# daooshee/ReReVST-Code

Measured on AMD Instinct MI355X. Metric: stylized frames/sec at 512x512, 1 style, higher is better.
Workload: dtype f32

## Files before the change

rerevst-code_amd/build.py:

```python
import os
import subprocess
import sys

HERE = os.path.dirname(os.path.abspath(__file__))
CSRC = os.path.join(HERE, "csrc")
LIB = os.path.join(HERE, "librerevst_hip.so")
SOURCES = ["rerevst_hip.hip"]
HEADERS = ["conv_mfma.h", "conv_wino.h", "conv_wino_split.h", "conv_f43.h", "conv_thin.h", "prep_kernels.h", "../../include/rerevst_hip.h"]


def _stale():
    if not os.path.exists(LIB):
        return True
    t = os.path.getmtime(LIB)
    return any(os.path.getmtime(os.path.join(CSRC, f)) > t for f in SOURCES + HEADERS)


def build_lib(force=False, verbose=True, extra=()):
    if not force and not _stale():
        return LIB
    hipcc = os.environ.get("HIPCC", "/opt/rocm/bin/hipcc")
    cmd = [hipcc, "--offload-arch=gfx950", "-O3", "-std=c++17", "-shared", "-fPIC",
           "-Wno-unused-result", *extra,
           *[os.path.join(CSRC, s) for s in SOURCES], "-o", LIB]
# ... 9 lines not shown
```

rerevst-code_amd/csrc/conv_wino.h:

```cpp
#pragma once
#include <hip/hip_runtime.h>
#include <stdint.h>
#include <utility>
#include <type_traits>
#include "conv_mfma.h"

#define WINO_PAR_BYTES 2048

template <int NW, int UPS, int SC = 0>
struct WinoGeo {
    static constexpr int NT = NW * 64;
    static constexpr int NB = NW == 8 ? 1 : 2;
    static constexpr int NP = UPS ? 9 : 16;
    static constexpr int NPU = NP + SC;
    static constexpr int PW = UPS ? 3 : 4;
    static constexpr int NPIECE = PW * PW;
    static constexpr int PPI = UPS ? 3 : 2;
    static constexpr int TIN = UPS ? 8 : 16;
    static constexpr int HALO = UPS ? 10 : 18;
    static constexpr int HALF = 18 * 9;
    static constexpr int PIECES = HALO * HALO * 4;
    static constexpr int RAW_IT = (PIECES + NT - 1) / NT;
    static constexpr int RAW_BYTES = RAW_IT * NT * 16;
    static constexpr int U_BYTES = NPU * 32 * 16 * 4;
    static constexpr int U_PIECES = U_BYTES / 16;
    static constexpr int U_IT = (U_PIECES + NT - 1) / NT;
    static constexpr int U_LDS = U_IT * NT * 16;
    static constexpr int SMEM = 2 * RAW_BYTES + 2 * U_LDS + WINO_PAR_BYTES;
    static constexpr int OCC = (UPS && NW == 4) ? 2 : 1;
// ... 83 lines not shown
    return r;
}
__device__ __forceinline__ f32x4 f4norm_clamp(const f32x4 v, const f32x4 m, const f32x4 r, const f32x4 lo, const f32x4 hi) {
    const f32x4 n = e4mul(f4sub(v, m), r);
    f32x4 o;
#pragma unroll
    for (int e = 0; e < 4; ++e) o[e] = med3(n[e], lo[e], hi[e]);
    return o;
}

template <class F, int... I>
__device__ __forceinline__ void static_for(F&& f, std::integer_sequence<int, I...>) {
    (f(std::integral_constant<int, I>{}), ...);
}

template <int EPI, int ABL = 0, int NW = 4, int UPS = 1, int SC = 0, int PERIMG = 0>
__global__ __launch_bounds__(NW * 64, (WinoGeo<NW, UPS, SC>::OCC)) void conv_wino_k(const ConvP p) {
    static_assert(UPS == 1 && NW == 4, "library kernel: upsample-fused form, 4 waves");
    static_assert(!(EPI & E_POOL), "no pooling behind an upsample");
    using G = WinoGeo<NW, UPS, SC>;
    constexpr int NPU = G::NPU;
    constexpr int RAW_BYTES = G::RAW_BYTES, U_BYTES = G::U_BYTES, U_LDS = G::U_LDS, NT = G::NT, NB = G::NB, NP = G::NP, PW = G::PW, NPIECE = G::NPIECE;
    extern __shared__ __attribute__((aligned(16))) char smem[];
    const int tid = threadIdx.x;
    const int wave = __builtin_amdgcn_readfirstlane(tid >> 6);
    const int lane = tid & 63, t = lane & 15, q = lane >> 4;
    const int tr = t >> 3, tc = t & 7;
    const int tg = wave;
    const int nchunks = p.Cin >> 4;
    const int n_ntiles = p.Cout >> 5;

    struct Item { int tx, ty, b, nt; };
    Item cur, nxt, dlt;
    {
        const int GD = gridDim.x, w = blockIdx.x;
// ... 100 lines not shown
        constexpr int PAR = decltype(par_c)::value;
        constexpr bool FIRST = decltype(first_c)::value;
        const bool own_u = c + 1 < nchunks, own_r = c + 2 < nchunks;
        const rsrc_t rs_u = make_rsrc(own_u ? w_t : w_n);
        const rsrc_t rs_ul = make_rsrc(own_u ? w_t : w_n, u_last_num);
        const rsrc_t rs_r = make_rsrc(own_r ? in_t : in_n);
        const rsrc_t rs_rl = make_rsrc(own_r ? in_t : in_n, raw_last_num);
        const int usoff = own_u ? (c + 1) * U_BYTES : 0;
        const int rsoff = (own_r ? c + 2 : c + 2 - nchunks) * 64;
        char* const udst = smem + 2 * RAW_BYTES + (1 - PAR) * U_LDS;
        char* const rdst = smem + PAR * RAW_BYTES;
        if (ABL & 128) {
            f32x4 u01[2] = {vcur[0], vcur[1]};
#pragma unroll
            for (int i = 0; i < NPU; ++i) {
                const f32x4 vv = vcur[i < NP ? i : 0];
#pragma unroll
                for (int s = 0; s < 4; ++s)
#pragma unroll
                    for (int nb = 0; nb < NB; ++nb)
                        acc[i][nb] = __builtin_amdgcn_mfma_f32_16x16x4f32(u01[nb][s], vv[s], (FIRST && s == 0) ? f32x4{0.f, 0.f, 0.f, 0.f} : acc[i][nb], 0, 0, 0);
            }
#pragma unroll
            for (int i = 0; i < NPIECE; ++i) vnext[i] = vcur[i];
            return;
        }
        const unsigned ub = PAR ? offU1 : offU;
        constexpr int RB = (1 - PAR) * RAW_BYTES;
        f32x4 u[4][NB];
        f32x4 (&d)[NPIECE] = vnext;
        u[0][0] = lds_rd128<0>(ub);
// ... 12 lines not shown
            }, std::make_integer_sequence<int, G::PPI>{});
            constexpr int cdx = i - 3;
            static_assert(G::col_iter(0) == 3 && G::col_iter(PW - 1) == PW + 2, "column release schedule");
            if constexpr (cdx >= 0 && cdx < PW) {
                asm volatile("s_waitcnt lgkmcnt(%5)" : "+v"(d[cdx * 3 + 0]), "+v"(d[cdx * 3 + 1]), "+v"(d[cdx * 3 + 2]), "+v"(u[i & 3][0]), "+v"(u[i & 3][1]) : "i"(G::younger(i)));
            } else {
                lds_release2<G::younger(i)>(u[i & 3][0], u[i & 3][1]);
            }
            __builtin_amdgcn_sched_barrier(0);
            if (!(ABL & 1)) {
                {
                    if constexpr (i < G::U_IT) bufld16_rs(i == G::U_IT - 1 ? rs_ul : rs_u, udst + (i * NT + wave * 64) * 16, tid * 16, usoff + i * NT * 16);
                    if constexpr (i < G::RAW_IT) bufld16_rs(i == G::RAW_IT - 1 ? rs_rl : rs_r, rdst + (i * NT + wave * 64) * 16, asrc[i], rsoff);
                }
            }
            const f32x4 vv = vcur[i < NP ? (i % PW) * PW + i / PW : 0];
#pragma unroll
            for (int s = 0; s < 4; ++s)
#pragma unroll
                for (int nb = 0; nb < NB; ++nb)
                    acc[i][nb] = __builtin_amdgcn_mfma_f32_16x16x4f32(u[i & 3][nb][s], vv[s], (FIRST && s == 0) ? f32x4{0.f, 0.f, 0.f, 0.f} : acc[i][nb], 0, 0, 0);
            static_for([&](auto xc) {
                constexpr int k = decltype(xc)::value;
                if constexpr (G::col_iter(k) == i) col_pass(d, k);
                if constexpr (G::row_iter(k) == i) row_pass(d, k);
            }, std::make_integer_sequence<int, PW>{});
        }, std::make_integer_sequence<int, NPU>{});
    };

    int par_ntile = -1, par_img = -1;
    long long tl[6] = {0, 0, 0, 0, 0, 0}, tl_t = 0;
// ... 53 lines not shown
        const int yb = e_y0 + 4 * tg + 2 * tr, xb = e_x0 + 2 * tc;
        f32x4 resv[NB][2][2];
        if (EPI & (E_RES | E_RES_UPS)) {
#pragma unroll
            for (int nb = 0; nb < NB; ++nb)
#pragma unroll
                for (int i = 0; i < 2; ++i)
#pragma unroll
                    for (int j = 0; j < 2; ++j) {
                        const int y = yb + i, x = xb + j;
                        const int ry = (EPI & E_RES_UPS) ? (y >> 1) : y, rx = (EPI & E_RES_UPS) ? (x >> 1) : x;
                        resv[nb][i][j] = f32x4{0.f, 0.f, 0.f, 0.f};
                        if (y < p.H && x < p.W)
                            resv[nb][i][j] = *(const f32x4*)(res_b + ((ry + 1) * (p.Wr + 2) + rx + 1) * p.Cout + e_ntile * 32 + nb * 16 + 4 * q);
                    }
        }
        if constexpr (SC) {
            const int ly = yb >> 1, lx = xb >> 1;
            if (ly < p.Hi && lx < p.Wi) {
                float* sc_b = p.sc_out + (size_t)e_b * (size_t)(p.Hi + 2) * (p.Wi + 2) * p.Cout + ((size_t)(ly + 1) * (p.Wi + 2) + lx + 1) * p.Cout;
#pragma unroll
                for (int nb = 0; nb < NB; ++nb) *(f32x4*)(sc_b + e_ntile * 32 + nb * 16 + 4 * q) = acc[NP][nb];
            }
        }
#pragma unroll
        for (int nb = 0; nb < NB; ++nb) {
            const int co = e_ntile * 32 + nb * 16 + 4 * q;
            f32x4 Y[2][2];
            f32x4 T[2][3];
#pragma unroll
            for (int c = 0; c < 3; ++c) {
                T[0][c] = acc[0 + c][nb] + acc[3 + c][nb];
                T[1][c] = acc[0 + c][nb] + acc[6 + c][nb];
            }
#pragma unroll
            for (int i = 0; i < 2; ++i) {
                Y[i][0] = T[i][0] + T[i][1];
                Y[i][1] = T[i][0] + T[i][2];
// ... 26 lines not shown
                        else if (p.out_p8) *(f32x4*)(out_b + (size_t)(co >> 3) * ((size_t)(p.H + 2) * (p.W + 8) * 8) + ((size_t)(y + 1) * (p.W + 8) + x + 4) * 8 + (co & 7)) = o;
                        else *(f32x4*)(out_b + ((y + 1) * (p.W + 2) + x + 1) * p.Cout + co) = o;
                    }
                }
        }
        tick(5);
    }
    asm volatile("s_waitcnt vmcnt(0)" ::: "memory");
    if ((ABL & 16) && lane == 0) {
        long long* dbg = p.dbg;
#pragma unroll
        for (int k = 0; k < 6; ++k) dbg[(blockIdx.x * NW + wave) * 6 + k] = tl[k];
    }
}

__global__ void pack_wino_k(const float* __restrict__ w, float* __restrict__ dst, int Cout, int Cin, int ups,
                            const float* __restrict__ wsc = nullptr) {
    constexpr int CH = 16;
    const int npt = ups ? 9 : 16, pw = ups ? 3 : 4;
    const int np = npt + (wsc ? 1 : 0);
    const size_t total = (size_t)Cout * Cin * np;
    for (size_t i = blockIdx.x * (size_t)blockDim.x + threadIdx.x; i < total; i += (size_t)gridDim.x * blockDim.x) {
        size_t r = i;
        const int cl = (int)(r % CH); r /= CH;
        const int j = r & 31; r >>= 5;
        const int pos = (int)(r % np); r /= np;
        const int nchunks = Cin / CH;
        const int chunk = r % nchunks; r /= nchunks;
        const int n_tile = (int)r;
        const int e = cl & 3, qs = cl >> 2;
        const int qq = qs ^ ((0 - (j >> 2)) & 3);
        const int co = n_tile * 32 + j, ci = chunk * CH + qq * 4 + e;
        if (pos >= npt) { dst[i] = wsc[(size_t)co * Cin + ci]; continue; }
        const float* g = w + ((size_t)co * Cin + ci) * 9;
        const int pr = pos / pw, pc = pos % pw;
        auto G3 = [&](int row, float g0, float g1, float g2) {
            if (ups) return row == 0 ? g0 + g1 + g2 : (row == 1 ? g0 : g2);
            return row == 0 ? g0 : (row == 1 ? 0.5f * (g0 + g1 + g2) : (row == 2 ? 0.5f * (g0 - g1 + g2) : g2));
        };
        float rowv[3];
#pragma unroll
        for (int kx = 0; kx < 3; ++kx) rowv[kx] = G3(pr, g[0 * 3 + kx], g[1 * 3 + kx], g[2 * 3 + kx]);
        dst[i] = G3(pc, rowv[0], rowv[1], rowv[2]);
    }
}
```

rerevst-code_amd/csrc/rerevst_hip.hip:

```cpp
#include <hip/hip_runtime.h>
#include <dlfcn.h>
#include <stddef.h>
#include <stdint.h>
#include <string.h>
#include <algorithm>
#include <cmath>
#include <thread>
#include <stdio.h>
#include <map>
#include <condition_variable>
#include <mutex>
#include <string>
#include <vector>

#include "../../include/rerevst_hip.h"
#include "conv_mfma.h"
#include "conv_wino.h"
#include "conv_wino_split.h"
#include "conv_f43.h"
#include "conv_thin.h"
#include "prep_kernels.h"

namespace {

// ... 380 lines not shown
    hipLaunchKernelGGL((conv_mfma_k<BN, TAPS, EPI>), grid, dim3(256), 0, s, p);
}

typedef void (*ConvFn)(const ConvP&, dim3, hipStream_t);
typedef hipError_t (*AttrFn)();
struct ConvKey { int BN, TAPS, UPS, EPI; ConvFn fn; const char* name; AttrFn attr; ConvFn fn_img = nullptr; };
#define CK(BN, TAPS, UPS, EPI) {BN, TAPS, UPS, EPI, &conv_launch<BN, TAPS, EPI>, "conv_mfma<" #BN "," #TAPS "," #EPI ">", nullptr}
const ConvKey CONV_TABLE[] = {
    CK(128, 1, 0, 0), CK(64, 1, 0, 0),
    CK(32, 9, 0, 0),
    CK(64, 9, 0, E_RELU | E_POOL), CK(128, 9, 0, E_RELU), CK(128, 9, 0, E_RELU | E_POOL), CK(128, 9, 0, E_RELU | E_NORM1),
};

constexpr int WINO_NW = 8;
constexpr int UPW_NW = 4;
template <int EPI, int NW, int UPS, int SC, int PERIMG = 0>
void wino_launch(const ConvP& p, dim3 grid, hipStream_t s) {
    using Geo = WinoGeo<NW, UPS, SC>;
    hipLaunchKernelGGL((conv_wino_k<EPI, 0, NW, UPS, SC, PERIMG>), grid, dim3(NW * 64), Geo::SMEM, s, p);
}
template <int EPI, int NW, int UPS, int SC, int PERIMG = 0>
hipError_t wino_attr() {
    hipError_t e = hipFuncSetAttribute((const void*)conv_wino_k<EPI, 0, NW, UPS, SC, 0>, hipFuncAttributeMaxDynamicSharedMemorySize, WinoGeo<NW, UPS, SC>::SMEM);
    if (e == hipSuccess && PERIMG) e = hipFuncSetAttribute((const void*)conv_wino_k<EPI, 0, NW, UPS, SC, 1>, hipFuncAttributeMaxDynamicSharedMemorySize, WinoGeo<NW, UPS, SC>::SMEM);
    return e;
}
template <int EPI, int PERIMG>
void wsplit_launch(const ConvP& p, dim3 grid, hipStream_t s) {
    hipLaunchKernelGGL((conv_wino_split_k<EPI, PERIMG>), grid, dim3(512), WSPLIT_SMEM_BYTES, s, p);
}
template <int EPI, int PERIMG>
hipError_t wsplit_attr() {
    hipError_t e = hipFuncSetAttribute((const void*)conv_wino_split_k<EPI, 0>, hipFuncAttributeMaxDynamicSharedMemorySize, WSPLIT_SMEM_BYTES);
    if (e == hipSuccess && PERIMG) e = hipFuncSetAttribute((const void*)conv_wino_split_k<EPI, 1>, hipFuncAttributeMaxDynamicSharedMemorySize, WSPLIT_SMEM_BYTES);
    return e;
}
template <int EPI, int LAY = 0>
void f43_launch(const ConvP& p, dim3 grid, hipStream_t s) {
    hipLaunchKernelGGL((conv_f43_k<EPI, LAY>), grid, dim3(F43Geo::NT), F43Geo::SMEM, s, p);
}
template <int EPI, int LAY = 0>
hipError_t f43_attr() { return hipFuncSetAttribute((const void*)conv_f43_k<EPI, LAY>, hipFuncAttributeMaxDynamicSharedMemorySize, F43Geo::SMEM); }
#define FK(EPI) {32, 9, 0, EPI, &f43_launch<EPI>, "conv_f43<" #EPI ">", &f43_attr<EPI>, nullptr}
struct F43LayKey { int EPI, LAY; ConvFn fn; const char* name; AttrFn attr; };
#define FKL(EPI, LAY) {EPI, LAY, &f43_launch<EPI, LAY>, "conv_f43<" #EPI ", " #LAY ">", &f43_attr<EPI, LAY>}
#define WK(EPI) {32, 9, 0, EPI, &wsplit_launch<EPI, 0>, "conv_wino<" #EPI ">", &wsplit_attr<EPI, 0>, nullptr}
#define WKI(EPI) {32, 9, 0, EPI, &wsplit_launch<EPI, 0>, "conv_wino<" #EPI ">", &wsplit_attr<EPI, 1>, &wsplit_launch<EPI, 1>}
#define UW(EPI) {32, 9, 1, EPI, &wino_launch<EPI, UPW_NW, 1, 0>, "conv_upw<" #EPI ">", &wino_attr<EPI, UPW_NW, 1, 0>}
#define UWS(EPI) {32, 10, 1, EPI, &wino_launch<EPI, UPW_NW, 1, 1>, "conv_upw_sc<" #EPI ">", &wino_attr<EPI, UPW_NW, 1, 1>}
#define UWSI(EPI) {32, 10, 1, EPI, &wino_launch<EPI, UPW_NW, 1, 1>, "conv_upw_sc<" #EPI ">", &wino_attr<EPI, UPW_NW, 1, 1, 1>, &wino_launch<EPI, UPW_NW, 1, 1, 1>}
const ConvKey WINO_TABLE[] = {
    WK(E_RELU), WK(E_RELU | E_POOL), WK(E_RELU | E_NORM1), WKI(E_LRELU | E_NORM1 | E_RES_UPS | E_NORM2), WKI(E_LRELU),
    WKI(0),
    WKI(E_RES), WKI(E_RES | E_NORM2),
    UW(E_LRELU | E_NORM1), UW(E_LRELU),
    UWSI(E_LRELU | E_NORM1),
    UWS(E_LRELU),
};

const ConvKey F43_TABLE[] = { FK(E_RELU), FK(E_RELU | E_POOL), FK(E_RELU | E_NORM1), FK(E_LRELU | E_NORM1 | E_RES_UPS | E_NORM2) };
const F43LayKey F43_LAY_TABLE[] = {
    FKL(E_RELU | E_POOL, 3), FKL(E_RELU, 3),
    FKL(E_RELU | E_POOL, 1),
    FKL(E_LRELU | E_NORM1 | E_RES_UPS | E_NORM2, 1),
};
// ... 26 lines not shown
int conv(rrv_handle h, const ConvCall& c) {
    const ConvW& w = *c.w;
    const ConvKey* k = nullptr;
    bool wino = false;
    bool f43 = !c.direct && use_f43(h, w, c.B, c.H, c.W, c.epi, c.ups, c.ksplit, c.bias_bstride != 0 || c.w_bstride != 0) &&
               !((c.wy0 | c.wx0 | c.wy1 | c.wx1) & 31);
    if (f43) {
        f43 = false;
        for (const ConvKey& e : F43_TABLE)
            if (e.EPI == c.epi) { k = &e; f43 = true; wino = true; break; }
    }
    const bool fuse_sc = c.ups && c.sc_out != nullptr;
    if (fuse_sc && !w.pk_ups_sc) return fail(h, RRV_E_ARG, "conv: no shortcut-fused pack for this layer");
    if (!f43 && !c.direct && (c.ups ? w.pk_ups != nullptr : w.pk_wino != nullptr)) {
        for (const ConvKey& e : WINO_TABLE)
            if (e.EPI == c.epi && e.UPS == (int)c.ups && (e.TAPS == 10) == fuse_sc) { k = &e; wino = true; break; }
    }
    const int ks = c.ksplit > 1 ? c.ksplit : 1;
    if (ks > 1 && !(wino && !c.ups && w.Cout == 32 && (w.Cin % (32 * ks)) == 0 && c.bias))
        return fail(h, RRV_E_ARG, "conv: split K needs the row-split kernel, a 32-cout layer, an even number of 16-channel chunks per slice and a split bias");
    if (!k && !c.ups) {
        for (const ConvKey& e : CONV_TABLE)
            if (e.BN == w.BN && e.TAPS == w.taps && e.EPI == c.epi) { k = &e; break; }
    }
    if (!k) {
        char b[128];
        snprintf(b, sizeof b, "no conv kernel for BN=%d taps=%d ups=%d epi=%d", w.BN, w.taps, (int)c.ups, c.epi);
        return fail(h, RRV_E_ARG, b);
    }
    const int lay = (c.in_p8 ? 1 : 0) | (c.out_p8 ? 2 : 0);
    ConvFn lay_fn = nullptr;
// ... 19 lines not shown
    p.par_bstride = c.par_bstride; p.bias_bstride = c.bias_bstride; p.w_bstride = c.w_bstride;
    if (ups_p8) { if (!wino) return fail(h, RRV_E_ARG, "conv: no upsample-fused kernel for this layer"); p.out_p8 = 1; }
    if ((c.par_bstride | c.bias_bstride || c.w_bstride) && !wino) return fail(h, RRV_E_ARG, "conv: per-image state needs a transform-domain kernel");
    if (c.ups && (c.bias_bstride || c.w_bstride)) return fail(h, RRV_E_ARG, "conv: the upsample-fused kernel shares weights and bias over the images of a launch");
    if (ks > 1) {
        p.Cin = w.Cin / ks; p.cstride = w.Cin; p.cin_slab_step = w.Cin / ks; p.Cout = 32 * ks;
    }
    if (c.res) { p.res = c.res->p; p.Hr = c.res->H; p.Wr = c.res->W; }
    p.tiles_x = (c.W + 15) / 16; p.tiles_y = (c.H + 7) / 8;
    if ((c.in_p8 ? c.in->C != 8 || c.in->B < c.B * (w.Cin / 8) : c.in->C != w.Cin) ||
        (c.out_p8 ? c.out->C != 8 || c.out->B < c.B * (w.Cout / 8) : c.out->C != w.Cout * ks)) return fail(h, RRV_E_ARG, "conv: channel mismatch");
    const int eh = c.ups ? c.H / 2 : c.H, ew = c.ups ? c.W / 2 : c.W;
    if (c.in->H != eh || c.in->W != ew + (c.in_p8 ? 6 : 0)) return fail(h, RRV_E_ARG, "conv: input geometry mismatch");
    const int oh = (c.epi & E_POOL) ? c.H / 2 : c.H, ow = (c.epi & E_POOL) ? c.W / 2 : c.W;
    if (c.out->H != oh || c.out->W != ow + (c.out_p8 ? 6 : 0)) return fail(h, RRV_E_ARG, "conv: output geometry mismatch");
    const int TS = f43 ? 32 : 16;
    if (wino) { p.tiles_x = (c.W + TS - 1) / TS; p.tiles_y = (c.H + TS - 1) / TS; }
    double win_frac = 1.0;
    if (wino && c.wy1 > c.wy0 && c.wx1 > c.wx0) {
        if ((c.wy0 | c.wx0 | c.wy1 | c.wx1) & 15) return fail(h, RRV_E_ARG, "conv: window must be tile aligned");
        p.ty0 = c.wy0 / TS; p.tx0 = c.wx0 / TS;
        p.tiles_y = (c.wy1 - c.wy0) / TS; p.tiles_x = (c.wx1 - c.wx0) / TS;
        win_frac = ((double)(c.wy1 - c.wy0) * (c.wx1 - c.wx0)) / ((double)((c.H + 15) / 16 * 16) * ((c.W + 15) / 16 * 16));
    }
    dim3 grid((unsigned)(p.tiles_x * p.tiles_y * c.B), (unsigned)(w.Cout / w.BN));
    if (wino) {
        const unsigned slabs = (unsigned)(w.Cout / 32) * ks;
        const unsigned items = (unsigned)(p.tiles_x * p.tiles_y * c.B) * slabs;
        const unsigned resident = resident_wgs(h, c.ups ? WinoGeo<UPW_NW, 1>::OCC : 1);
        grid = dim3(items < resident ? items : resident, 1);
        p.xcd_slabs = (grid.x % 8 == 0 && (grid.x / 8) % slabs == 0) ? 1 : 0;
    }
    const double px = (double)c.B * c.H * c.W * win_frac;
    const double cin = w.Cin;
    const double flops_sc = fuse_sc ? 2.0 * c.B * c.in->H * c.in->W * (double)w.Cout * cin : 0.0;
    const double flops = 2.0 * px * w.Cout * cin * w.taps + flops_sc;
    const double flops_exec = 2.0 * px * w.Cout * cin * (f43 ? 2.25 : wino ? (c.ups ? (fuse_sc ? 2.5 : 2.25) : 4.0) : (double)w.taps);
    const double bytes = 4.0 * ((double)c.B * c.in->H * c.in->W * cin + (double)c.B * oh * ow * w.Cout +
                                (c.res ? (double)c.B * c.res->H * c.res->W * w.Cout : 0.0) + (double)w.Cout * cin * w.taps +
                                (fuse_sc ? (double)c.B * c.in->H * c.in->W * w.Cout + (double)w.Cout * cin : 0.0));
    hipStream_t s = h->stream;
    ConvFn fn = lay_fn ? lay_fn : k->fn;
    if (wino && !f43 && (c.par_bstride | c.bias_bstride || c.w_bstride)) {
        if (!k->fn_img) return fail(h, RRV_E_ARG, "conv: this layer has no per-image-state kernel");
        fn = k->fn_img;
    }
    stamp(h, c.out, c.B);
    if (fuse_sc) stamp(h, c.sc_out, c.B);
    if (h->profiling) {
        char nm[160];
        snprintf(nm, sizeof nm, "%s@%dx%d@%dx%d", lay_name ? lay_name : k->name, w.Cin, w.Cout, c.H, c.W);
        return launch(h, nm, flops, bytes, [&] { fn(p, grid, s); }, flops_exec);
// ... 35 lines not shown
    hipLaunchKernelGGL(pack_f43_k, dim3(4096), dim3(256), 0, h->stream, (const float*)w.raw, w.pk_f43, w.Cout, w.Cin);
    HIPCHK(hipGetLastError());
    return RRV_OK;
}

int pack_ups(rrv_handle h, ConvW& w) {
    const size_t total = (size_t)w.Cout * w.Cin * 9;
    if (!w.pk_ups) RCHK(dalloc(h, &w.pk_ups, total, false));
    hipLaunchKernelGGL(pack_wino_k, dim3(4096), dim3(256), 0, h->stream, (const float*)w.raw, w.pk_ups, w.Cout, w.Cin, 1);
    HIPCHK(hipGetLastError());
    return RRV_OK;
}

int pack_ups_sc(rrv_handle h, ConvW& w, const ConvW& sc) {
    if (sc.Cout != w.Cout || sc.Cin != w.Cin || sc.taps != 1) return fail(h, RRV_E_WEIGHTS, "shortcut / conv1 shape mismatch");
    const size_t total = (size_t)w.Cout * w.Cin * 10;
    if (!w.pk_ups_sc) RCHK(dalloc(h, &w.pk_ups_sc, total, false));
    hipLaunchKernelGGL(pack_wino_k, dim3(4096), dim3(256), 0, h->stream, (const float*)w.raw, w.pk_ups_sc, w.Cout, w.Cin, 1, (const float*)sc.raw);
    HIPCHK(hipGetLastError());
    return RRV_OK;
}

int make_conv(rrv_handle h, const std::string& prefix, int cout, int cin, int taps, bool has_bias, bool do_pack = true) {
    ConvW w;
    w.Cout = cout; w.Cin = cin; w.taps = taps; w.BN = bn_for(cout);
    RCHK(upload(h, prefix + ".weight", &w.raw, (size_t)cout * cin * taps));
    if (has_bias) RCHK(upload(h, prefix + ".bias", &w.bias, (size_t)cout));
    else w.bias = h->zero_bias;
    if (do_pack) RCHK(pack(h, w));
    if (do_pack && taps == 9 && cin >= 64 && cout >= 64) RCHK(pack_wino(h, w));
    h->conv[prefix] = w;
    return RRV_OK;
}
// ... 2253 lines not shown
```

Before: 796.4.

## Add larger-tile Winograd kernel for upsample conv with fused shortcut

Adds a new kernel for the upsample conv that also carries the fused 1x1 shortcut. It uses a 4x4-input, 5x5-transform Winograd variant over 32-pixel output tiles, with 25 transform positions plus 4 for the shortcut. A new weight pack kernel lays out 26 weight blocks per chunk, and the host logic, tile size, window alignment and FLOP accounting change to match. The goal is fewer MFMA operations per output pixel. In exchange it holds many more accumulator registers and more LDS, and it rounds windows to 32-pixel alignment.

```diff
diff --git a/rerevst-code_amd/build.py b/rerevst-code_amd/build.py
--- a/rerevst-code_amd/build.py
+++ b/rerevst-code_amd/build.py
@@ -6,7 +6,7 @@
 CSRC = os.path.join(HERE, "csrc")
 LIB = os.path.join(HERE, "librerevst_hip.so")
 SOURCES = ["rerevst_hip.hip"]
-HEADERS = ["conv_mfma.h", "conv_wino.h", "conv_wino_split.h", "conv_f43.h", "conv_thin.h", "prep_kernels.h", "../../include/rerevst_hip.h"]
+HEADERS = ["conv_mfma.h", "conv_wino.h", "conv_ups5.h", "conv_wino_split.h", "conv_f43.h", "conv_thin.h", "prep_kernels.h", "../../include/rerevst_hip.h"]
 
 
 def _stale():
diff --git a/rerevst-code_amd/csrc/conv_ups5.h b/rerevst-code_amd/csrc/conv_ups5.h
--- /dev/null
+++ b/rerevst-code_amd/csrc/conv_ups5.h
@@ -0,0 +1,338 @@
+#pragma once
+
+struct Ups5Tab {
+    static constexpr int G2[5][3] = {{2, 0, 0}, {1, 1, 1}, {-1, -1, 1}, {-1, 1, 1}, {0, 0, 2}};
+    static constexpr int BT4[4][4] = {{1, 0, -1, 0}, {0, 1, 1, 0}, {0, -1, 1, 0}, {0, -1, 0, 1}};
+    static constexpr int AT[4][5] = {{1, 1, 0, -1, 0}, {0, 1, 1, 0, 0}, {0, 1, 0, 1, 0}, {0, 1, -1, 0, 1}};
+    static constexpr int DS[5] = {0, 1, 2, 2, 3};
+};
+template <int T, int R>
+constexpr int ups5_coef(int k) { return T == 0 ? Ups5Tab::BT4[R][k] : Ups5Tab::AT[R][k]; }
+template <int T, int R, int N>
+__device__ __forceinline__ f32x4 ups5_comb(const f32x4 (&x)[N]) {
+    constexpr int F = [] { for (int k = 0; k < N; ++k) if (ups5_coef<T, R>(k) == 1) return k; return -1; }();
+    static_assert(F >= 0, "every row has a +1 coefficient");
+    f32x4 r = x[F];
+    static_for([&](auto kc) {
+        constexpr int k = decltype(kc)::value;
+        constexpr int c = ups5_coef<T, R>(k);
+        static_assert(c == 0 || c == 1 || c == -1, "0 / +-1 coefficients");
+        if constexpr (k != F && c == 1) r = e4add(r, x[k]);
+        else if constexpr (c == -1) r = f4sub(r, x[k]);
+    }, std::make_integer_sequence<int, N>{});
+    return r;
+}
+
+struct Ups5Geo {
+    static constexpr int NT = 256, NB = 2;
+    static constexpr int NPOS = 29;
+    static constexpr int NUB = 26;
+    static constexpr int NPIECE = 16;
+    static constexpr int HALO = 18, HALF = 18 * 9;
+    static constexpr int PIECES = HALO * HALO * 4;
+    static constexpr int RAW_IT = (PIECES + NT - 1) / NT;
+    static constexpr int RAW_BYTES = RAW_IT * NT * 16;
+    static constexpr int U_BYTES = NUB * 32 * 16 * 4;
+    static constexpr int U_IT = U_BYTES / 16 / NT;
+    static_assert(U_IT * NT * 16 == U_BYTES, "U image is a whole number of LDS-DMA rounds");
+    static constexpr int SMEM = 2 * RAW_BYTES + 2 * U_BYTES + WINO_PAR_BYTES;
+    static_assert(SMEM <= 160 * 1024, "LDS");
+    static constexpr int OCC = 1;
+    static constexpr int vidx(int i) { return i < 25 ? Ups5Tab::DS[i % 5] * 4 + Ups5Tab::DS[i / 5] : (i == 25 ? 5 : i == 26 ? 9 : i == 27 ? 6 : 10); }
+    static constexpr int issued(int j) { return (j + 2 < NUB ? 2 : 0) + (j < NPIECE ? 1 : 0); }
+    static constexpr int younger(int i) {
+        return i == 0 ? 2 + issued(0) : i == 1 ? issued(0) + issued(1) : (i - 2 < NPIECE ? 1 : 0) + issued(i - 1) + issued(i);
+    }
+    static constexpr int col_iter(int dx) { return 4 * dx + 6; }
+    static constexpr int row_iter(int r) { return col_iter(3) + 1 + r; }
+};
+static_assert(Ups5Geo::row_iter(3) < Ups5Geo::NPOS, "next chunk transformed inside the MFMA loop");
+
+template <int EPI, int PERIMG>
+__device__ __forceinline__ void conv_ups5_body(const ConvP& p) {
+    static_assert(!(EPI & (E_POOL | E_RES | E_RES_UPS | E_NORM2)), "conv1 epilogues only: bias, activation, saved-stat normalise");
+    using G = Ups5Geo;
+    constexpr int RAW_BYTES = G::RAW_BYTES, U_BYTES = G::U_BYTES, NT = G::NT, NB = G::NB, NPOS = G::NPOS, NUB = G::NUB;
+    extern __shared__ __attribute__((aligned(16))) char smem[];
+    const int tid = threadIdx.x;
+    const int wave = __builtin_amdgcn_readfirstlane(tid >> 6);
+    const int lane = tid & 63, t = lane & 15, q = lane >> 4;
+    const int tr = t >> 3, tc = t & 7;
+    const int tg = wave;
+    const int nchunks = p.Cin >> 4;
+    const int n_ntiles = p.Cout >> 5;
+
+    struct Item { int tx, ty, b, nt; };
+    Item cur, nxt, dlt;
+    {
+        const int GD = gridDim.x, w = blockIdx.x;
+        int pix, dpix;
+        if (p.xcd_slabs) {
+            const int PT = (GD >> 3) / n_ntiles;
+            pix = (w & 7) * PT + (w >> 3) / n_ntiles; dpix = 8 * PT;
+            cur.nt = (w >> 3) % n_ntiles; dlt.nt = 0;
+        } else {
+            cur.nt = w % n_ntiles; pix = w / n_ntiles;
+            dlt.nt = GD % n_ntiles; dpix = GD / n_ntiles;
+        }
+        cur.tx = pix % p.tiles_x; cur.ty = (pix / p.tiles_x) % p.tiles_y; cur.b = pix / (p.tiles_x * p.tiles_y);
+        dlt.tx = dpix % p.tiles_x; dlt.ty = (dpix / p.tiles_x) % p.tiles_y; dlt.b = dpix / (p.tiles_x * p.tiles_y);
+    }
+    auto advance = [&](const Item& a) {
+        Item r = a;
+        r.nt += dlt.nt;
+        int carry = 0;
+        if (r.nt >= n_ntiles) { r.nt -= n_ntiles; carry = 1; }
+        r.tx += dlt.tx + carry;
+        if (r.tx >= p.tiles_x) { r.tx -= p.tiles_x; r.ty += 1; }
+        r.ty += dlt.ty;
+        if (r.ty >= p.tiles_y) { r.ty -= p.tiles_y; r.b += 1; }
+        r.b += dlt.b;
+        return r;
+    };
+    auto in_of = [&](const Item& a) {
+        return p.in + (size_t)a.b * (size_t)(p.Hi + 2) * (p.Wi + 2) * p.Cin + (size_t)(((a.ty + p.ty0) * 16) * (p.Wi + 2) + (a.tx + p.tx0) * 16) * p.Cin;
+    };
+    auto w_of = [&](const Item& a) { return p.wpk + (size_t)a.nt * nchunks * (NUB * 32 * 16); };
+    int asrc[G::RAW_IT];
+#pragma unroll
+    for (int it = 0; it < G::RAW_IT; ++it) {
+        const int e = it * NT + tid;
+        int P = e >> 2;
+        const int qq = e & 3;
+        if (P >= G::HALO * G::HALO) P = 0;
+        const int hf = P >= G::HALF, rem = P - hf * G::HALF;
+        const int hy = rem / 9, hx = 2 * (rem - hy * 9) + hf;
+        asrc[it] = ((hy * (p.Wi + 2) + hx) * p.Cin + 4 * (qq ^ ((hx >> 1) & 3))) * 4;
+    }
+    const int raw_last_num = ((G::RAW_IT - 1) * NT + wave * 64 < G::PIECES) ? 0x7fffffff : 0;
+    bool have = cur.b < p.B, have_nxt = false;
+    const float* in_t = in_of(cur);
+    const float* w_t = w_of(cur);
+    const float* in_n = in_t;
+    const float* w_n = w_t;
+    auto stage_u = [&](int chunk) {
+        char* udst = smem + 2 * RAW_BYTES + (chunk & 1) * U_BYTES;
+#pragma unroll
+        for (int it = 0; it < G::U_IT; ++it) bufld16(w_t, udst + (it * NT + wave * 64) * 16, tid * 16, chunk * U_BYTES + it * NT * 16);
+    };
+    auto stage_raw = [&](int chunk) {
+        char* rdst = smem + (chunk & 1) * RAW_BYTES;
+#pragma unroll
+        for (int it = 0; it < G::RAW_IT; ++it)
+            if (it * NT + wave * 64 < G::PIECES) bufld16(in_t, rdst + (it * NT + wave * 64) * 16, asrc[it], chunk * 64);
+    };
+    char* const par = smem + 2 * RAW_BYTES + 2 * U_BYTES;
+    auto stage_params = [&](int ntile, int img) {
+        if (wave < 2) {
+            const int e = tid;
+            const int row = e >> 3, col = (e & 7) * 4;
+            const float* src = p.bias;
+            const int pb = PERIMG ? img * p.par_bstride : 0;
+            int off = ntile * 32 + col;
+            if (row >= 1 && row <= 4) { src = (EPI & E_NORM1) ? p.n1 : p.bias; off = (EPI & E_NORM1) ? ntile * 32 + col + pb + (row - 1) * p.Cout : off; }
+            if (row > 4) { src = p.bias; off = ntile * 32; }
+            glds16(src + off, par + wave * 1024);
+        }
+    };
+
+    const unsigned lds0 = (unsigned)(size_t)(__attribute__((address_space(3))) char*)smem;
+    unsigned offD[4];
+#pragma unroll
+    for (int dx = 0; dx < 4; ++dx) {
+        const int hy = 4 * tg + 2 * tr, hx = 2 * tc + dx;
+        const int P = (hx & 1) * G::HALF + hy * 9 + (hx >> 1);
+        offD[dx] = lds0 + P * 64 + ((q ^ ((hx >> 1) & 3)) << 4);
+    }
+    const unsigned offU = lds0 + 2 * RAW_BYTES + t * 64 + ((q ^ ((0 - (t >> 2)) & 3)) << 4);
+    const unsigned offU1 = offU + U_BYTES;
+
+    f32x4 acc[NPOS][NB];
+    f32x4 va[16], vb[16];
+    auto pass = [](f32x4& x0, f32x4& x1, f32x4& x2, f32x4& x3) {
+        const f32x4 a[4] = {x0, x1, x2, x3};
+        x0 = ups5_comb<0, 0>(a); x1 = ups5_comb<0, 1>(a); x2 = ups5_comb<0, 2>(a); x3 = ups5_comb<0, 3>(a);
+    };
+    auto col_pass = [&](f32x4 (&d)[16], int dx) { pass(d[dx * 4 + 0], d[dx * 4 + 1], d[dx * 4 + 2], d[dx * 4 + 3]); };
+    auto row_pass = [&](f32x4 (&d)[16], int r) { pass(d[0 * 4 + r], d[1 * 4 + r], d[2 * 4 + r], d[3 * 4 + r]); };
+
+    auto chunk_body = [&](int c, auto par_c, auto first_c, f32x4 (&vcur)[16], f32x4 (&vnext)[16]) {
+        constexpr int PAR = decltype(par_c)::value;
+        constexpr bool FIRST = decltype(first_c)::value;
+        const bool own_u = c + 1 < nchunks, own_r = c + 2 < nchunks;
+        const rsrc_t rs_u = make_rsrc(own_u ? w_t : w_n);
+        const rsrc_t rs_r = make_rsrc(own_r ? in_t : in_n);
+        const rsrc_t rs_rl = make_rsrc(own_r ? in_t : in_n, raw_last_num);
+        const int usoff = own_u ? (c + 1) * U_BYTES : 0;
+        const int rsoff = (own_r ? c + 2 : c + 2 - nchunks) * 64;
+        char* const udst = smem + 2 * RAW_BYTES + (1 - PAR) * U_BYTES;
+        char* const rdst = smem + PAR * RAW_BYTES;
+        const unsigned ub = PAR ? offU1 : offU;
+        constexpr int RB = (1 - PAR) * RAW_BYTES;
+        f32x4 u[4][NB];
+        f32x4 (&d)[16] = vnext;
+        u[0][0] = lds_rd128<0>(ub);
+        u[0][1] = lds_rd128<1024>(ub);
+        u[1][0] = lds_rd128<2048>(ub);
+        u[1][1] = lds_rd128<2048 + 1024>(ub);
+        static_for([&](auto ic) {
+            constexpr int i = decltype(ic)::value;
+            if constexpr (i + 2 < NUB) {
+                u[(i + 2) & 3][0] = lds_rd128<(i + 2) * 2048>(ub);
+                u[(i + 2) & 3][1] = lds_rd128<(i + 2) * 2048 + 1024>(ub);
+            }
+            if constexpr (i < 16) d[i] = lds_rd128<RB + (i & 3) * 576>(offD[i >> 2]);
+            constexpr int US = (i < NUB ? i : NUB - 1) & 3;
+            if constexpr (i < NUB) {
+                constexpr int cdx = (i - 6) / 4;
+                if constexpr (i >= 6 && (i - 6) % 4 == 0 && cdx < 4) {
+                    static_assert(G::col_iter(cdx) == i, "column release schedule");
+                    asm volatile("s_waitcnt lgkmcnt(%6)" : "+v"(d[cdx * 4 + 0]), "+v"(d[cdx * 4 + 1]), "+v"(d[cdx * 4 + 2]), "+v"(d[cdx * 4 + 3]),
+                                 "+v"(u[US][0]), "+v"(u[US][1]) : "i"(G::younger(i)));
+                } else {
+                    lds_release2<G::younger(i)>(u[US][0], u[US][1]);
+                }
+            }
+            __builtin_amdgcn_sched_barrier(0);
+            if constexpr (i < G::U_IT) bufld16_rs(rs_u, udst + (i * NT + wave * 64) * 16, tid * 16, usoff + i * NT * 16);
+            if constexpr (i < G::RAW_IT) bufld16_rs(i == G::RAW_IT - 1 ? rs_rl : rs_r, rdst + (i * NT + wave * 64) * 16, asrc[i], rsoff);
+            const f32x4 vv = vcur[G::vidx(i)];
+#pragma unroll
+            for (int s = 0; s < 4; ++s)
+#pragma unroll
+                for (int nb = 0; nb < NB; ++nb)
+                    acc[i][nb] = __builtin_amdgcn_mfma_f32_16x16x4f32(u[US][nb][s], vv[s], (FIRST && s == 0) ? f32x4{0.f, 0.f, 0.f, 0.f} : acc[i][nb], 0, 0, 0);
+            static_for([&](auto xc) {
+                constexpr int k = decltype(xc)::value;
+                if constexpr (G::col_iter(k) == i) col_pass(d, k);
+                if constexpr (G::row_iter(k) == i) row_pass(d, k);
+            }, std::make_integer_sequence<int, 4>{});
+        }, std::make_integer_sequence<int, NPOS>{});
+    };
+
+    int par_ntile = -1, par_img = -1;
+    if (have) {
+        stage_raw(0);
+        stage_u(0);
+        stage_raw(1);
+        stage_params(cur.nt, cur.b);
+        par_ntile = cur.nt; par_img = cur.b;
+        __syncthreads();
+#pragma unroll
+        for (int k = 0; k < 16; ++k) va[k] = *(const f32x4*)(smem + (offD[k >> 2] - lds0) + (k & 3) * 576);
+#pragma unroll
+        for (int dx = 0; dx < 4; ++dx) col_pass(va, dx);
+#pragma unroll
+        for (int r = 0; r < 4; ++r) row_pass(va, r);
+        __syncthreads();
+    }
+    while (have) {
+        const int e_y0 = (cur.ty + p.ty0) * 32, e_x0 = (cur.tx + p.tx0) * 32, e_b = cur.b, e_ntile = cur.nt;
+        nxt = advance(cur);
+        have_nxt = nxt.b < p.B;
+        in_n = have_nxt ? in_of(nxt) : in_t;
+        w_n = have_nxt ? w_of(nxt) : w_t;
+        if (par_ntile != e_ntile || (PERIMG && par_img != e_b)) {
+            __syncthreads();
+            stage_params(e_ntile, e_b);
+            par_ntile = e_ntile; par_img = e_b;
+        }
+        chunk_body(0, std::integral_constant<int, 0>{}, std::true_type{}, va, vb);
+        __syncthreads();
+        chunk_body(1, std::integral_constant<int, 1>{}, std::false_type{}, vb, va);
+        __syncthreads();
+        for (int c = 2; c < nchunks; c += 2) {
+            chunk_body(c, std::integral_constant<int, 0>{}, std::false_type{}, va, vb);
+            __syncthreads();
+            chunk_body(c + 1, std::integral_constant<int, 1>{}, std::false_type{}, vb, va);
+            __syncthreads();
+        }
+        cur = nxt; have = have_nxt; in_t = in_n; w_t = w_n;
+
+        float* out_b = p.out + (size_t)e_b * (size_t)(p.H + 2) * (p.W + 2 + (p.out_p8 ? 6 : 0)) * p.Cout;
+        const int yb = e_y0 + 8 * tg + 4 * tr, xb = e_x0 + 4 * tc;
+        {
+            const int ly0 = yb >> 1, lx0 = xb >> 1;
+            float* sc_b = p.sc_out + (size_t)e_b * (size_t)(p.Hi + 2) * (p.Wi + 2) * p.Cout;
+#pragma unroll
+            for (int nb = 0; nb < NB; ++nb) {
+                const f32x4 s0 = f4sub(acc[25][nb], acc[27][nb]), s1 = e4add(acc[25][nb], acc[27][nb]);
+                const f32x4 t0 = f4sub(acc[26][nb], acc[28][nb]), t1 = e4add(acc[26][nb], acc[28][nb]);
+                const f32x4 sc[2][2] = {{f4sub(s0, t0), e4add(s0, t0)}, {f4sub(s1, t1), e4add(s1, t1)}};
+#pragma unroll
+                for (int a = 0; a < 2; ++a)
+#pragma unroll
+                    for (int b = 0; b < 2; ++b) {
+                        const int ly = ly0 + a, lx = lx0 + b;
+                        if (ly < p.Hi && lx < p.Wi)
+                            *(f32x4*)(sc_b + ((size_t)(ly + 1) * (p.Wi + 2) + lx + 1) * p.Cout + e_ntile * 32 + nb * 16 + 4 * q) = sc[a][b];
+                    }
+            }
+        }
+#pragma unroll
+        for (int nb = 0; nb < NB; ++nb) {
+            const int co = e_ntile * 32 + nb * 16 + 4 * q;
+            f32x4 T[5][4];
+#pragma unroll
+            for (int r = 0; r < 5; ++r) {
+                const f32x4 m[5] = {acc[r * 5 + 0][nb], acc[r * 5 + 1][nb], acc[r * 5 + 2][nb], acc[r * 5 + 3][nb], acc[r * 5 + 4][nb]};
+                T[r][0] = ups5_comb<1, 0>(m); T[r][1] = ups5_comb<1, 1>(m); T[r][2] = ups5_comb<1, 2>(m); T[r][3] = ups5_comb<1, 3>(m);
+            }
+            f32x4 Y[4][4];
+#pragma unroll
+            for (int j = 0; j < 4; ++j) {
+                const f32x4 tj[5] = {T[0][j], T[1][j], T[2][j], T[3][j], T[4][j]};
+                Y[0][j] = ups5_comb<1, 0>(tj); Y[1][j] = ups5_comb<1, 1>(tj); Y[2][j] = ups5_comb<1, 2>(tj); Y[3][j] = ups5_comb<1, 3>(tj);
+            }
+            const char* pl = par + (nb * 16 + 4 * q) * 4;
+            const f32x4 bias = *(const f32x4*)(pl);
+            f32x4 m1, r1, lo1, hi1;
+            if (EPI & E_NORM1) {
+                m1 = *(const f32x4*)(pl + 128); r1 = *(const f32x4*)(pl + 256);
+                lo1 = *(const f32x4*)(pl + 384); hi1 = *(const f32x4*)(pl + 512);
+            }
+#pragma unroll
+            for (int i = 0; i < 4; ++i)
+#pragma unroll
+                for (int j = 0; j < 4; ++j) {
+                    const int y = yb + i, x = xb + j;
+                    f32x4 o = e4add(Y[i][j], bias);
+                    if (EPI & E_RELU) o = f4relu(o);
+                    if (EPI & E_LRELU) o = f4lrelu(o);
+                    if (EPI & E_NORM1) o = f4norm_clamp(o, m1, r1, lo1, hi1);
+                    if (y < p.H && x < p.W) {
+                        if (p.out_p8) *(f32x4*)(out_b + (size_t)(co >> 3) * ((size_t)(p.H + 2) * (p.W + 8) * 8) + ((size_t)(y + 1) * (p.W + 8) + x + 4) * 8 + (co & 7)) = o;
+                        else *(f32x4*)(out_b + ((size_t)(y + 1) * (p.W + 2) + x + 1) * p.Cout + co) = o;
+                    }
+                }
+        }
+    }
+    asm volatile("s_waitcnt vmcnt(0)" ::: "memory");
+}
+
+__global__ void pack_ups5_k(const float* __restrict__ w, const float* __restrict__ wsc, float* __restrict__ dst, int Cout, int Cin) {
+    constexpr int CH = 16, NUB = Ups5Geo::NUB;
+    const size_t total = (size_t)Cout * Cin * NUB;
+    for (size_t i = blockIdx.x * (size_t)blockDim.x + threadIdx.x; i < total; i += (size_t)gridDim.x * blockDim.x) {
+        size_t r = i;
+        const int cl = (int)(r % CH); r /= CH;
+        const int j = r & 31; r >>= 5;
+        const int pos = (int)(r % NUB); r /= NUB;
+        const int nchunks = Cin / CH;
+        const int chunk = r % nchunks; r /= nchunks;
+        const int n_tile = (int)r;
+        const int e = cl & 3, qs = cl >> 2;
+        const int qq = qs ^ ((0 - (j >> 2)) & 3);
+        const int co = n_tile * 32 + j, ci = chunk * CH + qq * 4 + e;
+        if (pos == 25) { dst[i] = wsc[(size_t)co * Cin + ci] * 0.25f; continue; }
+        const float* g = w + ((size_t)co * Cin + ci) * 9;
+        auto G5 = [](int row, double g0, double g1, double g2) {
+            return 0.5 * (Ups5Tab::G2[row][0] * g0 + Ups5Tab::G2[row][1] * g1 + Ups5Tab::G2[row][2] * g2);
+        };
+        const int pr = pos / 5, pc = pos % 5;
+        double rowv[3];
+#pragma unroll
+        for (int kx = 0; kx < 3; ++kx) rowv[kx] = G5(pr, g[0 * 3 + kx], g[1 * 3 + kx], g[2 * 3 + kx]);
+        dst[i] = (float)G5(pc, rowv[0], rowv[1], rowv[2]);
+    }
+}
diff --git a/rerevst-code_amd/csrc/conv_wino.h b/rerevst-code_amd/csrc/conv_wino.h
--- a/rerevst-code_amd/csrc/conv_wino.h
+++ b/rerevst-code_amd/csrc/conv_wino.h
@@ -7,12 +7,12 @@
 
 #define WINO_PAR_BYTES 2048
 
-template <int NW, int UPS, int SC = 0>
+template <int NW, int UPS>
 struct WinoGeo {
     static constexpr int NT = NW * 64;
     static constexpr int NB = NW == 8 ? 1 : 2;
     static constexpr int NP = UPS ? 9 : 16;
-    static constexpr int NPU = NP + SC;
+    static constexpr int NPU = NP;
     static constexpr int PW = UPS ? 3 : 4;
     static constexpr int NPIECE = PW * PW;
     static constexpr int PPI = UPS ? 3 : 2;
@@ -126,11 +126,12 @@
     (f(std::integral_constant<int, I>{}), ...);
 }
 
-template <int EPI, int ABL = 0, int NW = 4, int UPS = 1, int SC = 0, int PERIMG = 0>
-__global__ __launch_bounds__(NW * 64, (WinoGeo<NW, UPS, SC>::OCC)) void conv_wino_k(const ConvP p) {
-    static_assert(UPS == 1 && NW == 4, "library kernel: upsample-fused form, 4 waves");
+#include "conv_ups5.h"
+
+template <int EPI, int ABL, int NW, int UPS, int PERIMG>
+__device__ __forceinline__ void conv_upw_body(const ConvP& p) {
     static_assert(!(EPI & E_POOL), "no pooling behind an upsample");
-    using G = WinoGeo<NW, UPS, SC>;
+    using G = WinoGeo<NW, UPS>;
     constexpr int NPU = G::NPU;
     constexpr int RAW_BYTES = G::RAW_BYTES, U_BYTES = G::U_BYTES, U_LDS = G::U_LDS, NT = G::NT, NB = G::NB, NP = G::NP, PW = G::PW, NPIECE = G::NPIECE;
     extern __shared__ __attribute__((aligned(16))) char smem[];
@@ -261,7 +262,7 @@
             f32x4 u01[2] = {vcur[0], vcur[1]};
 #pragma unroll
             for (int i = 0; i < NPU; ++i) {
-                const f32x4 vv = vcur[i < NP ? i : 0];
+                const f32x4 vv = vcur[i];
 #pragma unroll
                 for (int s = 0; s < 4; ++s)
 #pragma unroll
@@ -304,7 +305,7 @@
                     if constexpr (i < G::RAW_IT) bufld16_rs(i == G::RAW_IT - 1 ? rs_rl : rs_r, rdst + (i * NT + wave * 64) * 16, asrc[i], rsoff);
                 }
             }
-            const f32x4 vv = vcur[i < NP ? (i % PW) * PW + i / PW : 0];
+            const f32x4 vv = vcur[(i % PW) * PW + i / PW];
 #pragma unroll
             for (int s = 0; s < 4; ++s)
 #pragma unroll
@@ -388,14 +389,6 @@
                         if (y < p.H && x < p.W)
                             resv[nb][i][j] = *(const f32x4*)(res_b + ((ry + 1) * (p.Wr + 2) + rx + 1) * p.Cout + e_ntile * 32 + nb * 16 + 4 * q);
                     }
-        }
-        if constexpr (SC) {
-            const int ly = yb >> 1, lx = xb >> 1;
-            if (ly < p.Hi && lx < p.Wi) {
-                float* sc_b = p.sc_out + (size_t)e_b * (size_t)(p.Hi + 2) * (p.Wi + 2) * p.Cout + ((size_t)(ly + 1) * (p.Wi + 2) + lx + 1) * p.Cout;
-#pragma unroll
-                for (int nb = 0; nb < NB; ++nb) *(f32x4*)(sc_b + e_ntile * 32 + nb * 16 + 4 * q) = acc[NP][nb];
-            }
         }
 #pragma unroll
         for (int nb = 0; nb < NB; ++nb) {
@@ -452,11 +445,17 @@
     }
 }
 
-__global__ void pack_wino_k(const float* __restrict__ w, float* __restrict__ dst, int Cout, int Cin, int ups,
-                            const float* __restrict__ wsc = nullptr) {
+template <int EPI, int ABL = 0, int NW = 4, int UPS = 1, int SC = 0, int PERIMG = 0>
+__global__ __launch_bounds__(NW * 64, (SC ? Ups5Geo::OCC : WinoGeo<NW, UPS>::OCC)) void conv_wino_k(const ConvP p) {
+    static_assert(UPS == 1 && NW == 4, "library kernel: upsample-fused form, 4 waves");
+    if constexpr (SC) conv_ups5_body<EPI, PERIMG>(p);
+    else conv_upw_body<EPI, ABL, NW, UPS, PERIMG>(p);
+}
+
+__global__ void pack_wino_k(const float* __restrict__ w, float* __restrict__ dst, int Cout, int Cin, int ups) {
     constexpr int CH = 16;
     const int npt = ups ? 9 : 16, pw = ups ? 3 : 4;
-    const int np = npt + (wsc ? 1 : 0);
+    const int np = npt;
     const size_t total = (size_t)Cout * Cin * np;
     for (size_t i = blockIdx.x * (size_t)blockDim.x + threadIdx.x; i < total; i += (size_t)gridDim.x * blockDim.x) {
         size_t r = i;
@@ -469,7 +468,6 @@
         const int e = cl & 3, qs = cl >> 2;
         const int qq = qs ^ ((0 - (j >> 2)) & 3);
         const int co = n_tile * 32 + j, ci = chunk * CH + qq * 4 + e;
-        if (pos >= npt) { dst[i] = wsc[(size_t)co * Cin + ci]; continue; }
         const float* g = w + ((size_t)co * Cin + ci) * 9;
         const int pr = pos / pw, pc = pos % pw;
         auto G3 = [&](int row, float g0, float g1, float g2) {
diff --git a/rerevst-code_amd/csrc/rerevst_hip.hip b/rerevst-code_amd/csrc/rerevst_hip.hip
--- a/rerevst-code_amd/csrc/rerevst_hip.hip
+++ b/rerevst-code_amd/csrc/rerevst_hip.hip
@@ -418,15 +418,17 @@
 
 constexpr int WINO_NW = 8;
 constexpr int UPW_NW = 4;
+template <int NW, int UPS, int SC>
+constexpr int wino_smem() { return SC ? Ups5Geo::SMEM : WinoGeo<NW, UPS>::SMEM; }
 template <int EPI, int NW, int UPS, int SC, int PERIMG = 0>
 void wino_launch(const ConvP& p, dim3 grid, hipStream_t s) {
-    using Geo = WinoGeo<NW, UPS, SC>;
-    hipLaunchKernelGGL((conv_wino_k<EPI, 0, NW, UPS, SC, PERIMG>), grid, dim3(NW * 64), Geo::SMEM, s, p);
+    constexpr int smem = wino_smem<NW, UPS, SC>();
+    hipLaunchKernelGGL((conv_wino_k<EPI, 0, NW, UPS, SC, PERIMG>), grid, dim3(NW * 64), smem, s, p);
 }
 template <int EPI, int NW, int UPS, int SC, int PERIMG = 0>
 hipError_t wino_attr() {
-    hipError_t e = hipFuncSetAttribute((const void*)conv_wino_k<EPI, 0, NW, UPS, SC, 0>, hipFuncAttributeMaxDynamicSharedMemorySize, WinoGeo<NW, UPS, SC>::SMEM);
-    if (e == hipSuccess && PERIMG) e = hipFuncSetAttribute((const void*)conv_wino_k<EPI, 0, NW, UPS, SC, 1>, hipFuncAttributeMaxDynamicSharedMemorySize, WinoGeo<NW, UPS, SC>::SMEM);
+    hipError_t e = hipFuncSetAttribute((const void*)conv_wino_k<EPI, 0, NW, UPS, SC, 0>, hipFuncAttributeMaxDynamicSharedMemorySize, wino_smem<NW, UPS, SC>());
+    if (e == hipSuccess && PERIMG) e = hipFuncSetAttribute((const void*)conv_wino_k<EPI, 0, NW, UPS, SC, 1>, hipFuncAttributeMaxDynamicSharedMemorySize, wino_smem<NW, UPS, SC>());
     return e;
 }
 template <int EPI, int PERIMG>
@@ -451,8 +453,8 @@
 #define WK(EPI) {32, 9, 0, EPI, &wsplit_launch<EPI, 0>, "conv_wino<" #EPI ">", &wsplit_attr<EPI, 0>, nullptr}
 #define WKI(EPI) {32, 9, 0, EPI, &wsplit_launch<EPI, 0>, "conv_wino<" #EPI ">", &wsplit_attr<EPI, 1>, &wsplit_launch<EPI, 1>}
 #define UW(EPI) {32, 9, 1, EPI, &wino_launch<EPI, UPW_NW, 1, 0>, "conv_upw<" #EPI ">", &wino_attr<EPI, UPW_NW, 1, 0>}
-#define UWS(EPI) {32, 10, 1, EPI, &wino_launch<EPI, UPW_NW, 1, 1>, "conv_upw_sc<" #EPI ">", &wino_attr<EPI, UPW_NW, 1, 1>}
-#define UWSI(EPI) {32, 10, 1, EPI, &wino_launch<EPI, UPW_NW, 1, 1>, "conv_upw_sc<" #EPI ">", &wino_attr<EPI, UPW_NW, 1, 1, 1>, &wino_launch<EPI, UPW_NW, 1, 1, 1>}
+#define UWS(EPI) {32, 29, 1, EPI, &wino_launch<EPI, UPW_NW, 1, 1>, "conv_upw_sc<" #EPI ">", &wino_attr<EPI, UPW_NW, 1, 1>}
+#define UWSI(EPI) {32, 29, 1, EPI, &wino_launch<EPI, UPW_NW, 1, 1>, "conv_upw_sc<" #EPI ">", &wino_attr<EPI, UPW_NW, 1, 1, 1>, &wino_launch<EPI, UPW_NW, 1, 1, 1>}
 const ConvKey WINO_TABLE[] = {
     WK(E_RELU), WK(E_RELU | E_POOL), WK(E_RELU | E_NORM1), WKI(E_LRELU | E_NORM1 | E_RES_UPS | E_NORM2), WKI(E_LRELU),
     WKI(0),
@@ -509,7 +511,7 @@
     if (fuse_sc && !w.pk_ups_sc) return fail(h, RRV_E_ARG, "conv: no shortcut-fused pack for this layer");
     if (!f43 && !c.direct && (c.ups ? w.pk_ups != nullptr : w.pk_wino != nullptr)) {
         for (const ConvKey& e : WINO_TABLE)
-            if (e.EPI == c.epi && e.UPS == (int)c.ups && (e.TAPS == 10) == fuse_sc) { k = &e; wino = true; break; }
+            if (e.EPI == c.epi && e.UPS == (int)c.ups && (e.TAPS == 29) == fuse_sc) { k = &e; wino = true; break; }
     }
     const int ks = c.ksplit > 1 ? c.ksplit : 1;
     if (ks > 1 && !(wino && !c.ups && w.Cout == 32 && (w.Cin % (32 * ks)) == 0 && c.bias))
@@ -559,20 +561,27 @@
     if (c.in->H != eh || c.in->W != ew + (c.in_p8 ? 6 : 0)) return fail(h, RRV_E_ARG, "conv: input geometry mismatch");
     const int oh = (c.epi & E_POOL) ? c.H / 2 : c.H, ow = (c.epi & E_POOL) ? c.W / 2 : c.W;
     if (c.out->H != oh || c.out->W != ow + (c.out_p8 ? 6 : 0)) return fail(h, RRV_E_ARG, "conv: output geometry mismatch");
-    const int TS = f43 ? 32 : 16;
+    const int TS = f43 || fuse_sc ? 32 : 16;
     if (wino) { p.tiles_x = (c.W + TS - 1) / TS; p.tiles_y = (c.H + TS - 1) / TS; }
     double win_frac = 1.0;
     if (wino && c.wy1 > c.wy0 && c.wx1 > c.wx0) {
         if ((c.wy0 | c.wx0 | c.wy1 | c.wx1) & 15) return fail(h, RRV_E_ARG, "conv: window must be tile aligned");
-        p.ty0 = c.wy0 / TS; p.tx0 = c.wx0 / TS;
-        p.tiles_y = (c.wy1 - c.wy0) / TS; p.tiles_x = (c.wx1 - c.wx0) / TS;
-        win_frac = ((double)(c.wy1 - c.wy0) * (c.wx1 - c.wx0)) / ((double)((c.H + 15) / 16 * 16) * ((c.W + 15) / 16 * 16));
+        int wy0 = c.wy0, wx0 = c.wx0, wy1 = c.wy1, wx1 = c.wx1;
+        if (TS == 32 && !f43) {
+            wy0 &= ~31; wx0 &= ~31; wy1 = (wy1 + 31) & ~31; wx1 = (wx1 + 31) & ~31;
+            if (wy1 > ((c.H + 31) & ~31)) wy1 = (c.H + 31) & ~31;
+            if (wx1 > ((c.W + 31) & ~31)) wx1 = (c.W + 31) & ~31;
+        }
+        p.ty0 = wy0 / TS; p.tx0 = wx0 / TS;
+        p.tiles_y = (wy1 - wy0) / TS; p.tiles_x = (wx1 - wx0) / TS;
+        const int TD = fuse_sc ? 32 : 16;
+        win_frac = ((double)(wy1 - wy0) * (wx1 - wx0)) / ((double)((c.H + TD - 1) / TD * TD) * ((c.W + TD - 1) / TD * TD));
     }
     dim3 grid((unsigned)(p.tiles_x * p.tiles_y * c.B), (unsigned)(w.Cout / w.BN));
     if (wino) {
         const unsigned slabs = (unsigned)(w.Cout / 32) * ks;
         const unsigned items = (unsigned)(p.tiles_x * p.tiles_y * c.B) * slabs;
-        const unsigned resident = resident_wgs(h, c.ups ? WinoGeo<UPW_NW, 1>::OCC : 1);
+        const unsigned resident = resident_wgs(h, fuse_sc ? Ups5Geo::OCC : c.ups ? WinoGeo<UPW_NW, 1>::OCC : 1);
         grid = dim3(items < resident ? items : resident, 1);
         p.xcd_slabs = (grid.x % 8 == 0 && (grid.x / 8) % slabs == 0) ? 1 : 0;
     }
@@ -580,7 +589,7 @@
     const double cin = w.Cin;
     const double flops_sc = fuse_sc ? 2.0 * c.B * c.in->H * c.in->W * (double)w.Cout * cin : 0.0;
     const double flops = 2.0 * px * w.Cout * cin * w.taps + flops_sc;
-    const double flops_exec = 2.0 * px * w.Cout * cin * (f43 ? 2.25 : wino ? (c.ups ? (fuse_sc ? 2.5 : 2.25) : 4.0) : (double)w.taps);
+    const double flops_exec = 2.0 * px * w.Cout * cin * (f43 ? 2.25 : wino ? (c.ups ? (fuse_sc ? 29.0 / 16.0 : 2.25) : 4.0) : (double)w.taps);
     const double bytes = 4.0 * ((double)c.B * c.in->H * c.in->W * cin + (double)c.B * oh * ow * w.Cout +
                                 (c.res ? (double)c.B * c.res->H * c.res->W * w.Cout : 0.0) + (double)w.Cout * cin * w.taps +
                                 (fuse_sc ? (double)c.B * c.in->H * c.in->W * w.Cout + (double)w.Cout * cin : 0.0));
@@ -646,9 +655,9 @@
 
 int pack_ups_sc(rrv_handle h, ConvW& w, const ConvW& sc) {
     if (sc.Cout != w.Cout || sc.Cin != w.Cin || sc.taps != 1) return fail(h, RRV_E_WEIGHTS, "shortcut / conv1 shape mismatch");
-    const size_t total = (size_t)w.Cout * w.Cin * 10;
+    const size_t total = (size_t)w.Cout * w.Cin * Ups5Geo::NUB;
     if (!w.pk_ups_sc) RCHK(dalloc(h, &w.pk_ups_sc, total, false));
-    hipLaunchKernelGGL(pack_wino_k, dim3(4096), dim3(256), 0, h->stream, (const float*)w.raw, w.pk_ups_sc, w.Cout, w.Cin, 1, (const float*)sc.raw);
+    hipLaunchKernelGGL(pack_ups5_k, dim3(4096), dim3(256), 0, h->stream, (const float*)w.raw, (const float*)sc.raw, w.pk_ups_sc, w.Cout, w.Cin);
     HIPCHK(hipGetLastError());
     return RRV_OK;
 }
```

Result: faster. 862.2, median of 6 (+8.3%).
